# meijieru/AtomNAS

Hardware: AMD Instinct MI355X
Metric: images/sec (whole node) AtomNAS-C supernet 224x224 bs256/GPU (higher is better)
Workload: dtype bf16; 1 GPU; atomnas_c_supernet full training step (fwd + CE-smooth/L2/L1 + bwd + grad all-reduce + RMSprop + EMA), 224x224; per_gpu_batch=256, global_batch=256, parallelism=dp1, hip_graph=True

## Files before the change

### atomnas_amd/_lib.py

```python
import ctypes
import os

_HERE = os.path.dirname(os.path.abspath(__file__))
LIB_PATH = os.environ.get("ATOMNAS_HIP_LIB") or os.path.join(_HERE, "libatomnas_hip.so")

vp, i32, i64, f32, f64, u64 = (ctypes.c_void_p, ctypes.c_int, ctypes.c_long, ctypes.c_float, ctypes.c_double,
                               ctypes.c_ulonglong)

SIGNATURES = {
    "atomnas_dwconv_fwd": [vp, i32, i64, vp, vp, i32, vp, i32, vp, i32, i64, vp, i32, i32, i32, i32, i32, i32, i32, i32, i32, vp],
    "atomnas_dwconv_bwd": [vp, i32, i64, vp, i32, i64, vp, vp, vp, vp, i32, i64, vp, vp, i32, vp, i32, vp, i32, i64, vp, vp, i32, i32,
                           vp, i32, i32, i32, i32, i32, i32, i32, vp],
    "atomnas_pw_gemm_nt": [i32, vp, i32, i64, vp, i32, i64, vp, vp, vp, i32, vp, i32, vp, i32, i64, i32, vp, i32, vp, i32, i64, vp, vp,
                           i32, vp, vp, i32, i32, i64, i32, i32, i32, vp],
    "atomnas_pw_gemm_tn": [i32, vp, i32, i64, vp, i32, i64, vp, vp, vp, i32, i32, i32, vp, i32, i64, vp, i32, i64, vp, vp, vp, i32, i32,
                           vp, i64, i64, i64, vp, i64, i32, vp],
    "atomnas_expand_bwd": [vp, i32, i64, vp, vp, i32, vp, i32, vp, i32, vp, i32, vp, vp, i64, vp, i32, vp, i64, i32, i32, i32, vp],
    "atomnas_project_bwd": [vp, i32, vp, i32, vp, i32, i64, vp, vp, i32, vp, i32, i64, vp, i32, vp, i64, i64, vp, i64, i64, i32, i32, i32, vp],
    "atomnas_bn_finalize_fwd": [vp, i32, i32, f64, vp, vp, f32, f32, vp, vp, vp, vp, vp, vp, vp, i32, vp, vp],
    "atomnas_bn_eval_coeffs": [vp, vp, vp, vp, f32, vp, vp, i32, vp, vp],
    "atomnas_bn_finalize_bwd": [vp, i32, i32, f64, vp, vp, vp, vp, vp, vp, vp, vp, vp, vp, i32, vp, vp],
    "atomnas_bn_apply": [vp, i32, vp, vp, i32, vp, i32, vp, i32, i64, i32, i32, vp],
    "atomnas_bnbwd_apply": [vp, i32, vp, i32, vp, vp, vp, vp, i32, i64, i32, i32, vp],
    "atomnas_bn_act_pool": [vp, i32, vp, vp, i32, vp, i32, vp, f32, u64, vp, i32, i32, i32, i32, vp],
    "atomnas_pool_act_bwd": [vp, i32, vp, f32, vp, i32, vp, vp, i32, vp, i32, vp, i32, i32, i32, i32, i32, vp],
    "atomnas_act_bwd_stats": [vp, i32, vp, i32, vp, vp, i32, vp, i32, vp, i32, i64, i32, i32, vp],
    "atomnas_bn_apply_drop": [vp, i32, vp, vp, vp, i32, vp, i32, vp, f32, u64, vp, i32, i32, i32, i32, i32, vp],
    "atomnas_drop_connect_bwd": [vp, i32, vp, i32, vp, f32, vp, i32, vp, i32, i32, i32, i32, i32, vp],
    "atomnas_se_squeeze": [vp, i32, i64, vp, vp, i32, vp, i32, i32, i64, i32, i32, i32, i32, vp],
    "atomnas_se_mlp_fwd": [vp, i32, i32, i64, vp, vp, vp, vp, vp, vp, i32, vp, vp, i32, i32, i32, vp],
    "atomnas_se_scale": [vp, i32, i64, vp, vp, i32, vp, i32, vp, i32, i64, i64, i32, i32, i32, vp],
    "atomnas_se_bwd_gate": [vp, i32, i64, vp, i32, i64, vp, vp, i32, vp, vp, i32, vp, vp, vp, vp, vp, i32, i64, vp, vp, vp, vp, vp, vp, vp, i32, i32,
                            i32, i32, i32, i32, i32, vp],
    "atomnas_se_bwd_apply": [vp, i32, i64, vp, i32, i64, vp, vp, i32, vp, vp, i32, vp, i32, i64, vp, i32, i64, i32, i32, i32, vp],
    "atomnas_im2col_stem": [vp, vp, i32, i32, i32, i32, i32, vp],
    "atomnas_ce_smooth": [vp, i32, vp, f32, i32, i32, vp, vp, i32, f32, vp, i32, vp],
    "atomnas_colsum": [vp, i32, vp, i64, i32, i32, vp],
    "atomnas_fused_rmsprop_ema": [vp, vp, vp, vp, vp, vp, i64, vp, f64, f64, i32, f64, vp, vp, vp],
    "atomnas_fused_sgd_ema": [vp, vp, vp, vp, vp, i64, vp, f64, i32, vp, vp, vp],
    "atomnas_grad_guard": [vp, i64, vp, f32, i32, vp, vp, vp],
    "atomnas_fused_rmsprop_ema_guarded": [vp, vp, vp, vp, vp, vp, i64, vp, f64, f64, i32, f64, vp, vp, vp, vp],
    "atomnas_fused_sgd_ema_guarded": [vp, vp, vp, vp, vp, i64, vp, f64, i32, vp, vp, vp, vp],
    "atomnas_ema_update_guarded": [vp, vp, i64, vp, vp, vp],
    "atomnas_guard_restore": [vp, vp, i64, vp, i32, vp],
    "atomnas_vec_sum": [vp, i32, f32, vp, vp],
    "atomnas_ema_update": [vp, vp, i64, vp, vp],
    "atomnas_scale_by": [vp, i64, vp, i32, vp],
    "atomnas_accum_fold": [vp, vp, vp, i64, i32, i32, f32, vp],
    "atomnas_zero": [vp, i64, vp],
    "atomnas_add_i64": [vp, i64, i64, vp],
    "atomnas_reg_grad": [vp, vp, vp, i32, i32, vp, vp, vp],
    "atomnas_reg_value": [vp, vp, i32, i32, vp, f32, vp, vp, vp],
    "atomnas_pack_weights": [vp, vp, vp, i32, i32, vp],
    "atomnas_reduce_defer": [i32, vp],
    "atomnas_reduce_flush": [vp],
    "atomnas_gamma_mask": [vp, vp, vp, i32, f32, i32, vp, vp, vp, vp],
    "atomnas_mask_index": [vp, i32, vp, vp, vp],
    "atomnas_gather_dim": [vp, vp, vp, i64, i64, i64, i64, i32, i32, i32, vp],
    "atomnas_gather_jobs": [vp, i32, i64, vp],
    "atomnas_gram": [vp, i32, i64, i32, vp, i64, vp, vp, i32, vp],
    "atomnas_image_preprocess": [vp, vp, i32, i32, vp, vp, vp, i32, i32, vp],
    "atomnas_image_preprocess_large": [vp, vp, vp, i32, i32, i32, vp, vp, vp, i32, i32, vp, i64, vp],
    "atomnas_image_resize_window": [vp, vp, vp, i32, i32, vp, vp, vp, i32, i32, vp],
    "atomnas_image_resize_window_large": [vp, vp, vp, vp, i32, i32, i32, vp, vp, vp, i32, i32, vp, i64, vp],
    "atomnas_image_color": [vp, vp, i32, i32, vp, vp, vp, i32, vp, i32, vp],
    "atomnas_xb_coeffs": [vp, vp, vp, i32, vp, i32, vp, i32, i32, vp, i32, vp, vp, vp],
    "atomnas_fold_jobs": [vp, i32, i32, i64, i64, vp],
    "atomnas_block_infer": [vp, i32, vp, i32, vp, i32, vp, i32, vp, vp, vp, vp, vp, vp, vp, i32, i32, i32, i32, i32, i32, vp, vp, vp, i32, i32,
                            i32, i32, i32, vp],
    "atomnas_block_infer_se": [vp, i32, vp, i32, vp, i32, vp, i32, vp, vp, vp, vp, vp, vp, vp, i32, i32, i32, i32, i32, i32, vp, vp, vp, i32, i32,
                               i32, i32, i32, vp, vp, vp, vp, i32, i32, vp],
}
NO_STATUS = {"atomnas_last_error": (ctypes.c_char_p, []), "atomnas_abi_version": (i32, []),
             "atomnas_runtime_version": (i32, []), "atomnas_grad_guard_ws_floats": (i32, []), "atomnas_expand_bwd_supported": (i32, [i32, i32, i32]),
             "atomnas_project_bwd_supported": (i32, [i32, i32, i32]),
             "atomnas_project_bwd_dp_supported": (i32, [i64, i32, i32, i32, i32, i64, i32, i64, i32, i32]),
             "atomnas_dwconv_cw_supported": (i32, [i32, i32, i32, i32, i32, i32, i32, i32]),
             "atomnas_dwconv_mm_supported": (i32, [i32, i32, i32, i32, i32, i32, i32, i32]),
             "atomnas_se_pool_parts": (i32, [i32, i32, i32]),
             "atomnas_block_infer_supported": (i32, [i32, i32, i32, i32, i32, i32, vp, vp, vp, i32, i32, i32, i32, i32, i32]),
             "atomnas_block_infer_runs": (i32, [i32, i32, i32, i32, i32, i32, vp, vp, vp, i32, i32, i32, i32, i32, i32]),
             "atomnas_block_infer_se_supported": (i32, [i32, i32, i32, i32, i32, i32, vp, vp, vp, i32, i32, i32, i32, i32, i32]),
             "atomnas_block_infer_se_runs": (i32, [i32, i32, i32, i32, i32, i32, vp, vp, vp, i32, i32, i32, i32, i32, i32])}

ABI_VERSION = 9
_lib = None


class AtomnasHipError(RuntimeError):
    pass


def exported_symbols():
    return sorted(list(SIGNATURES) + list(NO_STATUS))


def load():
    global _lib
    if _lib is not None:
        return _lib
    import torch
    if not os.path.exists(LIB_PATH):
        raise AtomnasHipError(
            "libatomnas_hip.so is missing (%s). Build it with `python -m atomnas_amd.build`; there is no CPU fallback." % LIB_PATH)
    lib = ctypes.CDLL(LIB_PATH)
    for name, args in SIGNATURES.items():
        fn = getattr(lib, name)
        fn.argtypes = args
        fn.restype = i32
    for name, (res, args) in NO_STATUS.items():
        fn = getattr(lib, name)
        fn.argtypes = args
        fn.restype = res
    if lib.atomnas_abi_version() != ABI_VERSION:
        raise AtomnasHipError("%s has ABI version %d, this package binds version %d: rebuild with `python -m atomnas_amd.build`"
                              % (LIB_PATH, lib.atomnas_abi_version(), ABI_VERSION))
    _lib = lib
    return lib


PROFILE = None
_TAG = [None]


def profile_tag(tag):
    _TAG[0] = tag


def call(name, *args):
    lib = load()
    if PROFILE is not None:
        import torch
        e0, e1 = torch.cuda.Event(enable_timing=True), torch.cuda.Event(enable_timing=True)
        e0.record()
        rc = getattr(lib, name)(*args)
        e1.record()
        PROFILE.append((name, _TAG[0], e0, e1))
    else:
        rc = getattr(lib, name)(*args)
    if rc != 0:
        raise AtomnasHipError("%s failed (rc=%d): %s" % (name, rc, lib.atomnas_last_error().decode()))
```

### atomnas_amd/csrc/head.hip

```cpp
#include "common.h"

namespace atomnas {

template <typename T>
__global__ __launch_bounds__(256) void k_im2col_stem(const float* __restrict__ img, T* __restrict__ col, int ld, int N, int H, int W,
                                                     int Ho, int Wo) {
  const long total = (long)N * Ho * Wo;
  for (long m = (long)blockIdx.x * 256 + threadIdx.x; m < total; m += (long)gridDim.x * 256) {
    const int wo = (int)(m % Wo), ho = (int)((m / Wo) % Ho), n = (int)(m / ((long)Wo * Ho));
    float v[32];
#pragma unroll
    for (int i = 0; i < 32; ++i) v[i] = 0.f;
#pragma unroll
    for (int ci = 0; ci < 3; ++ci) {
      const float* plane = img + ((long)n * 3 + ci) * H * W;
#pragma unroll
      for (int ky = 0; ky < 3; ++ky) {
        const int hi = 2 * ho + ky - 1;
#pragma unroll
        for (int kx = 0; kx < 3; ++kx) {
          const int wi = 2 * wo + kx - 1;
          if (hi >= 0 && hi < H && wi >= 0 && wi < W) v[ci * 9 + ky * 3 + kx] = plane[(long)hi * W + wi];
        }
      }
    }
    T* o = col + m * ld;
#pragma unroll
    for (int g8 = 0; g8 < 4; ++g8) {
      float t[8];
#pragma unroll
      for (int e = 0; e < 8; ++e) t[e] = v[8 * g8 + e];
      VecIO<T, 8>::store(o + 8 * g8, t);
    }
    const float z8[8] = {0.f, 0.f, 0.f, 0.f, 0.f, 0.f, 0.f, 0.f};
    for (int c = 32; c < ld; c += 8) VecIO<T, 8>::store(o + c, z8);
  }
}

template <typename T>
__global__ __launch_bounds__(256) void k_ce_smooth(const float* __restrict__ logits, int ldl, const long long* __restrict__ target,
                                                   float eps, int B, int K, float* __restrict__ loss_per_sample,
                                                   T* __restrict__ dlogits, int ldd, float gscale,
                                                   int* __restrict__ topk_correct ) {
  const int lane = threadIdx.x & 63;
  const int b = blockIdx.x * 4 + (threadIdx.x >> 6);
  if (b >= B) return;
  const float* x = logits + (long)b * ldl;
  const int y = (int)target[b];
  float mx = -INFINITY;
  for (int j = lane; j < K; j += 64) mx = fmaxf(mx, x[j]);
#pragma unroll
  for (int o = 32; o > 0; o >>= 1) mx = fmaxf(mx, __shfl_xor(mx, o, 64));
  float se = 0.f, sx = 0.f;
  const float xy = x[y];
  int rank = 0;
  for (int j = lane; j < K; j += 64) {
    const float v = x[j];
    se += expf(v - mx);
    sx += v;
    rank += (v > xy) ? 1 : 0;
  }
  se = wave_sum(se);
  sx = wave_sum(sx);
#pragma unroll
  for (int o = 32; o > 0; o >>= 1) rank += __shfl_xor(rank, o, 64);
  const float lse = mx + logf(se);
  const float loss = -(1.f - eps) * (xy - lse) - (eps / (float)K) * (sx - (float)K * lse);
  if (lane == 0) {
    if (loss_per_sample) loss_per_sample[b] = loss;
    if (topk_correct) {
      if (rank < 1) atomicAdd(&topk_correct[0], 1);
      if (rank < 5) atomicAdd(&topk_correct[1], 1);
    }
  }
  if (dlogits) {
    T* d = dlogits + (long)b * ldd;
    const float invB = gscale / (float)B;
    for (int j = lane; j < ldd; j += 64) {
      float g = 0.f;
      if (j < K) {
        const float p = expf(x[j] - lse);
        const float t = eps / (float)K + ((j == y) ? (1.f - eps) : 0.f);
        g = (p - t) * invB;
      }
      d[j] = from_f32<T>(g);
    }
  }
}

template <typename T>
__global__ __launch_bounds__(256) void k_colsum(const T* __restrict__ x, int ld, float* __restrict__ out, long M, int C) {
  const int c = blockIdx.x * 256 + threadIdx.x;
  if (c >= C) return;
  float s0 = 0.f, s1 = 0.f, s2 = 0.f, s3 = 0.f;
  long m = 0;
  for (; m + 3 < M; m += 4) {
    s0 += to_f32(x[m * ld + c]);
    s1 += to_f32(x[(m + 1) * ld + c]);
    s2 += to_f32(x[(m + 2) * ld + c]);
    s3 += to_f32(x[(m + 3) * ld + c]);
  }
  for (; m < M; ++m) s0 += to_f32(x[m * ld + c]);
  out[c] += (s0 + s1) + (s2 + s3);
}

}

using namespace atomnas;

extern "C" int atomnas_im2col_stem(const float* img, void* col, int ld, int N, int H, int W, int dtype, void* stream) {
  ATOMNAS_REQUIRE(img && col && ld >= 32 && ld % 8 == 0 && N > 0 && H > 0 && W > 0, "im2col_stem: bad arguments");
  const int Ho = (H + 2 - 3) / 2 + 1, Wo = (W + 2 - 3) / 2 + 1;
  const long total = (long)N * Ho * Wo;
  long blocks = (total + 255) / 256;
  if (blocks > 8192) blocks = 8192;
  hipStream_t st = (hipStream_t)stream;
  if (dtype == DT_F32)
    hipLaunchKernelGGL(k_im2col_stem<float>, dim3((unsigned)blocks), dim3(256), 0, st, img, (float*)col, ld, N, H, W, Ho, Wo);
  else
    hipLaunchKernelGGL(k_im2col_stem<bf16_t>, dim3((unsigned)blocks), dim3(256), 0, st, img, (bf16_t*)col, ld, N, H, W, Ho, Wo);
  return check_launch("im2col_stem");
}

extern "C" int atomnas_ce_smooth(const float* logits, int ldl, const long long* target, float eps, int B, int K, float* loss_per_sample,
                                 void* dlogits, int ldd, float gscale, int* topk_correct, int dtype, void* stream) {
  ATOMNAS_REQUIRE(logits && target && B > 0 && K > 0 && ldl >= K, "ce_smooth: bad arguments");
  ATOMNAS_REQUIRE(!dlogits || ldd >= K, "ce_smooth: bad gradient pitch");
  hipStream_t st = (hipStream_t)stream;
  if (dtype == DT_F32)
    hipLaunchKernelGGL(k_ce_smooth<float>, dim3((B + 3) / 4), dim3(256), 0, st, logits, ldl, target, eps, B, K, loss_per_sample,
                       (float*)dlogits, ldd, gscale, topk_correct);
  else
    hipLaunchKernelGGL(k_ce_smooth<bf16_t>, dim3((B + 3) / 4), dim3(256), 0, st, logits, ldl, target, eps, B, K, loss_per_sample,
                       (bf16_t*)dlogits, ldd, gscale, topk_correct);
  return check_launch("ce_smooth");
}

extern "C" int atomnas_colsum(const void* x, int ld, float* out, long M, int C, int dtype, void* stream) {
  ATOMNAS_REQUIRE(x && out && M > 0 && C > 0 && ld >= C, "colsum: bad arguments");
  dim3 grid((C + 255) / 256);
  hipStream_t st = (hipStream_t)stream;
  if (dtype == DT_F32) hipLaunchKernelGGL(k_colsum<float>, grid, dim3(256), 0, st, (const float*)x, ld, out, M, C);
  else hipLaunchKernelGGL(k_colsum<bf16_t>, grid, dim3(256), 0, st, (const bf16_t*)x, ld, out, M, C);
  return check_launch("colsum");
}
```

### atomnas_amd/functional.py

```python
import os

import torch
from torch import nn

from . import ops
from .ops import PRO_BNBWD, PRO_BNRELU, PRO_NONE, STAT_SQ, STAT_Z
from .ops import Slab
from .runtime import pad8, pads

ACT_NONE, ACT_RELU, ACT_RELU6, ACT_SWISH = 0, 1, 2, 3


def act_code(module):
    if module is None:
        return ACT_NONE
    if isinstance(module, nn.ReLU6):
        return ACT_RELU6
    if isinstance(module, nn.ReLU):
        return ACT_RELU
    if type(module).__name__ == "Swish":
        return ACT_SWISH
    raise NotImplementedError("activation %s is not supported by the HIP path (ReLU / ReLU6 / Swish)" % type(module).__name__)


# ... 367 lines not shown
    @staticmethod
    def backward(ctx, gout):
        pl, sv = ctx.pl, ctx.sv
        G, _ = to_2d(gout, pl.mgr.compute_dtype)
        N, H, W, _, _ = sv["dims"]
        gx = block_backward(pl, sv, G)
        _stap(pl, gx=gx)
        ctx.sv = None
        pl.mgr.grad_done(pl)
        return to_4d(gx, N, H, W, pl.inp), None, None


def run_block(pl, x, anchor):
    if pl.nb == 0:
        return x
    if torch.is_grad_enabled() and (x.requires_grad or anchor.requires_grad):
        return BlockFunction.apply(x, anchor, pl)
    x2d, (N, H, W, C) = to_2d(x, pl.mgr.compute_dtype)
    out, _ = block_forward(pl, x2d, N, H, W, False)
    s = pl.stride
    return to_4d(out, N, (H - 1) // s + 1, (W - 1) // s + 1, pl.oup)


class SEFunction(torch.autograd.Function):

    @staticmethod
    def forward(ctx, x, w1, b1, w2, b2, se_act, dtype):
        x2d, (N, H, W, C) = to_2d(x, dtype)
        dev = x.device
        hid = w1.shape[0]
        HT = pads(C)
        M = N * H * W
        D = ops.zeros(M, HT, dtype=dtype, device=dev)
        D[:, :C] = x2d
        cmap = torch.full((HT,), -1, dtype=torch.int32, device=dev)
        cmap[:C] = torch.arange(C, dtype=torch.int32, device=dev)
        w1p, w2t, b2p = (ops.zeros(*shape, dtype=torch.float32, device=dev) for shape in ((hid, HT), (hid, HT), (HT,)))
        w1p[:, :C] = w1.detach().reshape(hid, C).float()
        w2t[:, :C] = w2.detach().reshape(C, hid).float().t()
        b2p[:C] = b2.detach().float()
        one, zero = torch.ones(HT, dtype=torch.float32, device=dev), ops.zeros(HT, dtype=torch.float32, device=dev)
        one[C:] = 0
        S = torch.empty(M, HT, dtype=dtype, device=dev)
        sv = _se_forward(D, one, zero, ACT_NONE, S, cmap, w1p, b1.detach().float().contiguous(), w2t, b2p, se_act, hid, N, H * W, HT)
        ctx.save_for_backward(D, one, zero, sv["gate"], sv["pooled"], cmap, w1p, w2t, sv["hpre"])
        ctx.dims = (N, H, W, C, HT, hid, se_act, dtype)
        return to_4d(S[:, :C], N, H, W, C)

    @staticmethod
    def backward(ctx, gout):
        D, one, zero, gate, pooled, cmap, w1p, w2t, hpre = ctx.saved_tensors
        N, H, W, C, HT, hid, se_act, dtype = ctx.dims
        dev = D.device
        M = N * H * W
        g2d, _ = to_2d(gout, dtype)
        dS = ops.zeros(M, HT, dtype=dtype, device=dev)
        dS[:, :C] = g2d
        dw1, db1, dw2, db2 = (_f32(hid * C, dev, zero=True), _f32(hid, dev, zero=True), _f32(C * hid, dev, zero=True), _f32(C, dev, zero=True))
        g = torch.empty(M, HT, dtype=dtype, device=dev)
        _se_backward(dS, D, one, zero, ACT_NONE, dict(gate=gate, pooled=pooled, hpre=hpre), cmap, w1p, w2t, se_act, hid, dw1, db1, dw2, db2,
                     C, g, _stats(HT, dev), N, H * W, HT)
        return (to_4d(g[:, :C], N, H, W, C), dw1.view(hid, C, 1, 1), db1, dw2.view(C, hid, 1, 1), db2, None, None)


def run_se(module, x):
    dtype = x.dtype if x.dtype in (torch.float32, torch.bfloat16) else torch.float32
    return SEFunction.apply(x, module.se_reduce.weight, module.se_reduce.bias, module.se_expand.weight, module.se_expand.bias,
                            act_code(module.active_fn), dtype)


def convbn_forward(pl, x, need_grad):
    mgr = pl.mgr
    T = mgr.compute_dtype
    dev = x.device
    act = pl.act
    sv = {}
    if pl.groups == 1 and pl.k == 3:
        if pl.cin != 3 or pl.stride != 2:
            raise NotImplementedError("dense 3x3 convolution other than the 3-channel stride-2 stem")
        N, _, H, W = x.shape
        Ho, Wo = (H - 1) // 2 + 1, (W - 1) // 2 + 1
        M = N * Ho * Wo
        col = torch.empty(M, 32, dtype=T, device=dev)
        ops.im2col_stem(x.float().contiguous(), col, N, H, W)
        a2d, K = col, 27
        sv["kind"] = "stem"
    elif pl.groups == 1 and pl.k == 1:
        a2d, (N, H, W, C) = to_2d(x, T)
        Ho, Wo, M, K = H, W, N * H * W, pl.cin
        sv["kind"] = "pw"
    else:
        a2d, (N, H, W, C) = to_2d(x, T)
        s = pl.stride
        Ho, Wo = (H - 1) // s + 1, (W - 1) // s + 1
        M = N * Ho * Wo
        sv["kind"] = "dw"
    Cp = pad8(pl.cout)
    Y = torch.empty(M, Cp, dtype=T, device=dev) if sv["kind"] != "dw" else ops.zeros(M, Cp, dtype=T, device=dev)
    st = _stats(pl.cout, dev, pl.bn["mgr"]) if bn_uses_batch_stats(pl.bn) else None
    if sv["kind"] == "dw":
        ops.dwconv_fwd(a2d, None, None, 0, pl.taps, Y, stat_ld=pl.cout, N=N, H=H, W=W, C=pl.cout, k=pl.k, stride=pl.stride,
                       **_fwd_stats(st, mode=False))
    else:
        ops.gemm_nt(a2d, pl.W_pack, Y, M, pl.cout, K, **_fwd_stats(st))
    b = bn_forward_coeffs(pl.bn, st, M, dev)
    if act:
        _tap("convbn", pl, Y, b)
    out = torch.empty(M, Cp, dtype=T, device=dev)
    ops.bn_apply(Y, b.scale, b.shift, int(act), None, out, M, pl.cout)
    _stap(pl, Y=Y, bn=b, out=out)
    if need_grad:
        sv.update(a=a2d, Y=Y, b=b, dims=(N, H, W, Ho, Wo), K=K if sv["kind"] != "dw" else 0)
    return out, (N, Ho, Wo), sv


def convbn_backward(pl, sv, G, need_input_grad):
    dev, T = G.device, G.dtype
    N, H, W, Ho, Wo = sv["dims"]
    M = N * Ho * Wo
    act = pl.act
    Y, b, a2d = sv["Y"], sv["b"], sv["a"]
    g = torch.empty_like(Y)
    st2 = _stats(pl.cout, dev, pl.bn["mgr"])
    ops.act_bwd_stats(G, Y, b.scale if act else None, b.shift if act else None, int(act), g, st2.t, M, pl.cout, stat_rows=st2.rows)
    c1, c2, c3 = bn_backward_coeffs(pl.bn, b, st2, M, dev)
    _stap(pl, g=g, c=(c1, c2, c3))
    if sv["kind"] == "dw":
        h = ops.zeros(N * H * W, pad8(pl.cout), dtype=T, device=dev)
        ops.dwconv_bwd(g, Y, c1, c2, c3, a2d, None, None, 0, pl.taps, h, pl.W_grad, None, 0, N, H, W, pl.cout, pl.k, pl.stride)
        return h
    K = sv["K"]
    ops.gemm_tn(a2d, K, g, pl.cout, pl.W_grad, 1, K, M, v_mode=PRO_BNBWD, v2=Y, vc1=c1, vc2=c2, vc3=c3)
    if not need_input_grad or sv["kind"] == "stem":
        return None
    Gx = torch.empty(M, pad8(K), dtype=T, device=dev)
    ops.gemm_nt(g, pl.WT_pack, Gx, M, K, pl.cout, a_mode=PRO_BNBWD, a2=Y, ac1=c1, ac2=c2, ac3=c3)
    return Gx


class ConvBNFunction(torch.autograd.Function):
    @staticmethod
    def forward(ctx, x, anchor, pl):
        out, (N, Ho, Wo), sv = convbn_forward(pl, x, True)
        ctx.pl, ctx.sv = pl, sv
        ctx.x_needs = x.requires_grad
        return to_4d(out[:, :pl.cout] if out.shape[1] != pl.cout else out, N, Ho, Wo, pl.cout)

    @staticmethod
    def backward(ctx, gout):
        pl, sv = ctx.pl, ctx.sv
        G, _ = to_2d(gout, pl.mgr.compute_dtype)
        gx = convbn_backward(pl, sv, G, ctx.x_needs)
        ctx.sv = None
        pl.mgr.grad_done(pl)
        N, H, W, _, _ = sv["dims"]
        if gx is None:
            return None, None, None
        cin = pl.cin
        return to_4d(gx[:, :cin] if gx.shape[1] != cin else gx, N, H, W, cin), None, None


def run_convbn(pl, x, anchor):
    if pl.cout % 8 != 0:
        raise ValueError("ConvBNReLU output channels must be a multiple of 8 on the HIP path, got %d" % pl.cout)
    if torch.is_grad_enabled() and (x.requires_grad or anchor.requires_grad):
        return ConvBNFunction.apply(x, anchor, pl)
    out, (N, Ho, Wo), _ = convbn_forward(pl, x, False)
    return to_4d(out, N, Ho, Wo, pl.cout)


def tail_forward(lp, fp, x, drop_p, training, seed, step_ptr, need_grad):
    mgr = lp.mgr
    T = mgr.compute_dtype
    dev = x.device
    a2d, (N, H, W, C) = to_2d(x, T)
    M = N * H * W
    act = lp.act
    L = torch.empty(M, lp.cout, dtype=T, device=dev)
    st = _stats(lp.cout, dev, lp.bn["mgr"]) if bn_uses_batch_stats(lp.bn) else None
    ops.gemm_nt(a2d, lp.W_pack, L, M, lp.cout, lp.cin, **_fwd_stats(st))
    b = bn_forward_coeffs(lp.bn, st, M, dev)
    if act:
        _tap("convbn", lp, L, b)
    pooled = torch.empty(N, lp.cout, dtype=T, device=dev)
    p = float(drop_p) if training else 0.0
# ... 118 lines not shown
```

### atomnas_amd/ops.py

```python
import ctypes

import os

import torch

from . import _lib
from ._lib import call

PRO_NONE, PRO_BNRELU, PRO_BNBWD = 0, 1, 2
STAT_NONE, STAT_SQ, STAT_Z = 0, 1, 2
HYP_LR, HYP_RHO, HYP_EMA_DECAY, HYP_GRAD_SCALE = 0, 1, 2, 3


RECORD = None


def _lay(t):
    if t is None:
        return None
    return "slab" if isinstance(t, Slab) else int(t.stride(0))


def _rec(entry, **kw):
    if RECORD is not None:
# ... 357 lines not shown
         _p(p_scale), _p(p_shift), int(N), int(H), int(W), int(inp), int(oup), n, _ints(seg_off), _ints(seg_ch), _ints(seg_k), int(stride), int(act),
         int(bool(expand)), int(bool(residual)), dt_code(x.dtype), *se_args, _stream())


def bnbwd_apply(g, x, c1, c2, c3, y, M, C):
    _chk_cuda(g, x, y)
    _rec("bnbwd_apply", M=int(M), C=int(C), g=_lay(g), x=_lay(x), y=_lay(y), dt=dt_code(g.dtype))
    call("atomnas_bnbwd_apply", _p(g), _ld(g), _p(x), _ld(x), _p(c1), _p(c2), _p(c3), _p(y), _ld(y), M, C, dt_code(g.dtype), _stream())


def bn_act_pool(x, scale, shift, relu, pooled, keep, drop_p, seed, step_ptr, N, HW, C):
    _rec("bn_act_pool", N=int(N), HW=int(HW), C=int(C), x=_lay(x), act=int(relu), drop_p=float(drop_p), keep=keep is not None, dt=dt_code(x.dtype))
    call("atomnas_bn_act_pool", _p(x), _ld(x), _p(scale), _p(shift), int(relu), _p(pooled), _ld(pooled), _p(keep), float(drop_p),
         int(seed) & 0xFFFFFFFFFFFFFFFF, _p(step_ptr), N, HW, C, dt_code(x.dtype), _stream())


def pool_act_bwd(dpooled, keep, drop_p, x, scale, shift, relu, g, stats2, N, HW, C, stat_rows=None):
    _rec("pool_act_bwd", N=int(N), HW=int(HW), C=int(C), x=_lay(x), act=int(relu), drop_p=float(drop_p), keep=keep is not None,
         stat_rows=_rows(stats2, stat_rows), dt=dt_code(x.dtype))
    call("atomnas_pool_act_bwd", _p(dpooled), _ld(dpooled), _p(keep), float(drop_p), _p(x), _ld(x), _p(scale), _p(shift), int(relu),
         _p(g), _ld(g), _p(stats2), _rows(stats2, stat_rows), N, HW, C, dt_code(x.dtype), _stream())


def act_bwd_stats(dy, z, scale, shift, relu, g, stats2, M, C, stat_rows=None):
    _rec("act_bwd_stats", M=int(M), C=int(C), dy=_lay(dy), z=_lay(z), masked=scale is not None, act=int(relu), g=_lay(g), stat_rows=_rows(stats2, stat_rows),
         dt=dt_code(dy.dtype))
    call("atomnas_act_bwd_stats", _p(dy), _ld(dy), _p(z), _ld(z), _p(scale), _p(shift), int(relu), _p(g),
         _ld(g) if g is not None else 0, _p(stats2), _rows(stats2, stat_rows), M, C, dt_code(dy.dtype), _stream())


def bn_apply_drop(x, scale, shift, res, y, keep_out, drop_p, seed, step_ptr, block_index, N, HW, C):
    _chk_cuda(x, res, y, keep_out)
    _rec("bn_apply_drop", N=int(N), HW=int(HW), C=int(C), x=_lay(x), res=_lay(res), y=_lay(y), drop_p=float(drop_p), block=int(block_index),
         dt=dt_code(x.dtype))
    call("atomnas_bn_apply_drop", _p(x), _ld(x), _p(scale), _p(shift), _p(res), _ld(res) if res is not None else 0, _p(y), _ld(y), _p(keep_out), float(drop_p),
         int(seed) & 0xFFFFFFFFFFFFFFFF, _p(step_ptr), int(block_index), N, HW, C, dt_code(x.dtype), _stream())


def drop_connect_bwd(g, z, keep, drop_p, gs, stats2, N, HW, C, stat_rows=None):
    _chk_cuda(g, z, keep, gs)
    _rec("drop_connect_bwd", N=int(N), HW=int(HW), C=int(C), g=_lay(g), z=_lay(z), gs=_lay(gs), drop_p=float(drop_p),
         stat_rows=_rows(stats2, stat_rows), dt=dt_code(g.dtype))
    call("atomnas_drop_connect_bwd", _p(g), _ld(g), _p(z), _ld(z), _p(keep), float(drop_p), _p(gs), _ld(gs), _p(stats2),
         _rows(stats2, stat_rows), N, HW, C, dt_code(g.dtype), _stream())


def se_pool_parts(N, HW, C):
    return int(_lib.load().atomnas_se_pool_parts(int(N), int(HW), int(C)))


def se_squeeze(d, scale, shift, act, pooled_parts, N, HW, C):
    parts = pooled_parts.shape[0]
    call("atomnas_se_squeeze", _p(d), _ld(d), _ss(d), _p(scale), _p(shift), int(act), _p(pooled_parts), pooled_parts.stride(1), parts,
         pooled_parts.stride(0), N, HW, C, dt_code(d.dtype), _stream())


def se_mlp_fwd(pooled_parts, pooled, cmap, w1p, b1, w2t, b2p, act, hpre, gate, N, HT, hid):
    call("atomnas_se_mlp_fwd", _p(pooled_parts), pooled_parts.stride(1), pooled_parts.shape[0], pooled_parts.stride(0), _p(pooled), _p(cmap),
         _p(w1p), _p(b1), _p(w2t), _p(b2p), int(act), _p(hpre), _p(gate), N, HT, hid, _stream())


def se_scale(d, scale, shift, act, gate, out, M, HW, C):
    call("atomnas_se_scale", _p(d), _ld(d), _ss(d), _p(scale), _p(shift), int(act), _p(gate), gate.stride(0), _p(out), _ld(out), _ss(out), M,
         HW, C, dt_code(d.dtype), _stream())


def se_bwd_gate(ds, d, scale, shift, act, gate, pooled, cmap, w1p, w2t, hpre,
                dgate, dz2, dz1, dpooled, dw1, db1, dw2, db2, N, HW, HT, total,
                hid, se_act=None):
    call("atomnas_se_bwd_gate", _p(ds), _ld(ds), _ss(ds), _p(d), _ld(d), _ss(d), _p(scale), _p(shift), int(act), _p(gate), _p(pooled),
         gate.stride(0), _p(cmap), _p(w1p), _p(w2t), _p(hpre), _p(dgate), dgate.shape[0], dgate.stride(0), _p(dz2), _p(dz1), _p(dpooled), _p(dw1), _p(db1), _p(dw2), _p(db2),
         int(act if se_act is None else se_act), N, HW, HT, total, hid, dt_code(d.dtype), _stream())


def se_bwd_apply(ds, d, scale, shift, act, gate, dpooled, g, stats2, M, HW, C, stat_rows=None):
    call("atomnas_se_bwd_apply", _p(ds), _ld(ds), _ss(ds), _p(d), _ld(d), _ss(d), _p(scale), _p(shift), int(act), _p(gate), _p(dpooled),
         gate.stride(0), _p(g), _ld(g), _ss(g), _p(stats2), _rows(stats2, stat_rows), M, HW, C, dt_code(d.dtype), _stream())


def im2col_stem(img, col, N, H, W):
    assert img.dtype == torch.float32 and img.is_contiguous()
    _rec("im2col_stem", N=int(N), H=int(H), W=int(W), col=_lay(col), dt=dt_code(col.dtype))
    call("atomnas_im2col_stem", _p(img), _p(col), _ld(col), N, H, W, dt_code(col.dtype), _stream())


def ce_smooth(logits, target, eps, B, K, loss_per_sample, dlogits, gscale, topk):
    assert logits.dtype == torch.float32 and target.dtype == torch.int64
    _rec("ce_smooth", B=int(B), K=int(K), ldl=_lay(logits), dl=_lay(dlogits), dt=dt_code(dlogits.dtype) if dlogits is not None else 0)
    call("atomnas_ce_smooth", _p(logits), _ld(logits), _p(target), float(eps), B, K, _p(loss_per_sample), _p(dlogits),
         _ld(dlogits) if dlogits is not None else 0, float(gscale), _p(topk),
         dt_code(dlogits.dtype) if dlogits is not None else 0, _stream())


def colsum(x, out, M, C):
    _rec("colsum", M=int(M), C=int(C), x=_lay(x), dt=dt_code(x.dtype))
    call("atomnas_colsum", _p(x), _ld(x), _p(out), M, C, dt_code(x.dtype), _stream())


def fused_rmsprop_ema(p, g, sq, buf, ema, wd_chunk, n, hyper, alpha, eps, eps_inside_sqrt, momentum, l2_value=None, ws=None, guard=None):
    if l2_value is not None and ws is None:
        ws = torch.empty(4096, dtype=torch.float32, device=p.device)
    args = (_p(p), _p(g), _p(sq), _p(buf), _p(ema), _p(wd_chunk), n, _p(hyper), float(alpha), float(eps), int(eps_inside_sqrt),
            float(momentum), _p(l2_value), _p(ws))
    if guard is None:
        call("atomnas_fused_rmsprop_ema", *args, _stream())
    else:
        call("atomnas_fused_rmsprop_ema_guarded", *args, _p(guard), _stream())


def fused_sgd_ema(p, g, buf, ema, wd_chunk, n, hyper, momentum, nesterov, l2_value=None, ws=None, guard=None):
    if l2_value is not None and ws is None:
        ws = torch.empty(4096, dtype=torch.float32, device=p.device)
    args = (_p(p), _p(g), _p(buf), _p(ema), _p(wd_chunk), n, _p(hyper), float(momentum), int(bool(nesterov)), _p(l2_value), _p(ws))
    if guard is None:
        call("atomnas_fused_sgd_ema", *args, _stream())
    else:
        call("atomnas_fused_sgd_ema_guarded", *args, _p(guard), _stream())


GUARD_OK, GUARD_SCALE, GUARD_NORM, GUARD_COEF, GUARD_SKIPPED, GUARD_CLIPPED = 0, 1, 2, 3, 4, 5
GUARD_WORDS = 8


def grad_guard_ws_floats():
    return int(_lib.load().atomnas_grad_guard_ws_floats())


def grad_guard(g, n, hyper, max_norm, skip_nonfinite, guard, ws=None):
    if ws is None:
        ws = torch.empty(grad_guard_ws_floats(), dtype=torch.float32, device=g.device)
    assert guard.dtype == torch.float32 and guard.numel() >= GUARD_WORDS and ws.numel() >= grad_guard_ws_floats()
    call("atomnas_grad_guard", _p(g), int(n), _p(hyper), float(max_norm), int(bool(skip_nonfinite)), _p(ws), _p(guard), _stream())


def ema_update_guarded(shadow, x, n, hyper, guard):
    call("atomnas_ema_update_guarded", _p(shadow), _p(x), n, _p(hyper), _p(guard), _stream())


def guard_restore(dst, src, n, guard, unconditional=False):
    call("atomnas_guard_restore", _p(dst), _p(src), int(n), _p(guard), int(bool(unconditional)), _stream())


def vec_sum(x, n, scale, out):
    call("atomnas_vec_sum", _p(x), int(n), float(scale), _p(out), _stream())


def ema_update(shadow, x, n, hyper):
    call("atomnas_ema_update", _p(shadow), _p(x), n, _p(hyper), _stream())


def zero_(t):
    if isinstance(t, Slab):
        zero_(t.t)
        return t
    assert t.is_contiguous()
    if t.numel():
        call("atomnas_zero", _p(t), t.numel() * t.element_size(), _stream())
    return t


def zeros(*shape, dtype, device):
    return zero_(torch.empty(*shape, dtype=dtype, device=device))


def add_i64(t, v):
    assert t.dtype == torch.int64 and t.is_contiguous()
# ... 147 lines not shown
```

### include/atomnas_hip.h

```cpp
#ifndef ATOMNAS_HIP_H
#define ATOMNAS_HIP_H

#ifdef __cplusplus
extern "C" {
#endif

#define ATOMNAS_STAT_ROWS_DEFAULT 512

#define ATOMNAS_DT_F32 0
#define ATOMNAS_DT_BF16 1

#define ATOMNAS_ACT_NONE 0
#define ATOMNAS_ACT_RELU 1
#define ATOMNAS_ACT_RELU6 2
#define ATOMNAS_ACT_SWISH 3

#define ATOMNAS_PRO_NONE 0
#define ATOMNAS_PRO_BNRELU 1
#define ATOMNAS_PRO_BNBWD 2

#define ATOMNAS_STAT_NONE 0
#define ATOMNAS_STAT_SQ 1
#define ATOMNAS_STAT_Z 2

// ... 15 lines not shown
int atomnas_runtime_version(void);

int atomnas_dwconv_fwd(const void* x, int ldx, long x_ss, const float* in_scale, const float* in_shift, int in_relu, const float* w,
                       int ldw, void* y, int ldy, long y_ss, float* stats, int stat_ld, int stat_rows, int N, int H, int W, int C, int k, int stride,
                       int dtype, void* stream);

int atomnas_dwconv_bwd(const void* g, int ldg, long g_ss, const void* yraw, int ldyr, long yraw_ss, const float* c1, const float* c2,
                       const float* c3, const void* x, int ldx, long x_ss, const float* in_scale, const float* in_shift, int in_relu,
                       const float* w, int ldw, void* h, int ldh, long h_ss, float* dw, float* stats, int stat_ld, int part_rows, float* dw_ws, int N, int H, int W,
                       int C, int k, int stride, int dtype, void* stream);

int atomnas_dwconv_cw_supported(int N, int H, int W, int C, int k, int stride, int dtype, int dir);

int atomnas_dwconv_mm_supported(int N, int H, int W, int C, int k, int stride, int dtype, int dir);

int atomnas_pw_gemm_nt(int a_mode, const void* a, int lda, long a_ss, const void* a2, int lda2, long a2_ss, const float* ac1,
                       const float* ac2, const float* ac3, int a_relu, const void* wp, int ldw, void* c, int ldc, long c_ss, int out_f32,
                       const void* add, int ldadd, const void* z, int ldz, long z_ss, const float* zscale, const float* zshift, int mask, const float* bias,
                       float* stats, int stat_mode, int stat_rows, long M, int N, int K, int dtype, void* stream);

int atomnas_pw_gemm_tn(int u_mode, const void* u, int ldu, long u_ss, const void* u2, int ldu2, long u2_ss, const float* uc1,
                       const float* uc2, const float* uc3, int u_relu, int NU, int v_mode, const void* v, int ldv, long v_ss,
                       const void* v2, int ldv2, long v2_ss, const float* vc1, const float* vc2, const float* vc3, int v_relu, int NV, float* out, long si, long sj, long M,
                       float* ws, long ws_floats, int dtype, void* stream);

int atomnas_expand_bwd_supported(int inp, int hid, int dtype);
int atomnas_expand_bwd(const void* h, int ldh, long h_ss, const float* c1, const void* x, int ldx, const void* wt, int ldw, const void* add,
                       int ldadd, void* gx, int ldgx, float* dwe, float* ws, long ws_floats, const void* mp, int ldm, const float* vb, long M,
                       int inp, int hid, int dtype, void* stream);
int atomnas_gram(const void* x, int ldx, long M, int inp, float* ws, long ws_floats, float* gram, float* sx, int dtype, void* stream);
int atomnas_xb_coeffs(const float* c2, const float* c3, const void* wexp, int ldwe, const float* gram, int ldg, const float* sx, int inp,
                      int C, void* mp, int ldm, float* vb, float* dwe, void* stream);

int atomnas_project_bwd_supported(int oup, int hid, int dtype);
int atomnas_project_bwd_dp_supported(long M, int oup, int hid, int ldg, int ldz, long z_ss, int ldgh, long gh_ss, int stat_rows, int dtype);
int atomnas_project_bwd(const void* g, int ldg, const void* wpt, int ldw, const void* z, int ldz, long z_ss, const float* zscale,
                        const float* zshift, int act, void* gh, int ldgh, long gh_ss, float* stats, int stat_rows, float* dwp, long si,
                        long sj, float* ws, long ws_floats, long M, int oup, int hid, int dtype, void* stream);

int atomnas_bn_finalize_fwd(const float* stats, int stat_rows, int stat_ld, double count, const float* gamma, const float* beta, float eps, float momentum,
                            float* running_mean, float* running_var, long long* num_batches_tracked, float* scale, float* shift,
                            float* save_mean, float* save_invstd, int C, const int* cmap, void* stream);
int atomnas_bn_eval_coeffs(const float* gamma, const float* beta, const float* running_mean, const float* running_var, float eps,
                           float* scale, float* shift, int C, const int* cmap, void* stream);
int atomnas_bn_finalize_bwd(const float* stats2, int stat_rows, int stat_ld, double count, const float* gamma, const float* save_mean, const float* save_invstd,
                            const float* rho_ptr, const float* penalty, float* dgamma, float* dbeta, float* c1, float* c2, float* c3,
                            int C, const int* cmap, void* stream);
int atomnas_bn_apply(const void* x, int ldx, const float* scale, const float* shift, int relu, const void* res, int ldres, void* y,
                     int ldy, long M, int C, int dtype, void* stream);
int atomnas_bnbwd_apply(const void* g, int ldg, const void* x, int ldx, const float* c1, const float* c2, const float* c3, void* y,
                        int ldy, long M, int C, int dtype, void* stream);
int atomnas_bn_act_pool(const void* x, int ldx, const float* scale, const float* shift, int relu, void* pooled, int ldp,
                        unsigned char* keep, float drop_p, unsigned long long seed, const long long* step_ptr, int N, int HW, int C,
                        int dtype, void* stream);
int atomnas_pool_act_bwd(const void* dpooled, int ldp, const unsigned char* keep, float drop_p, const void* x, int ldx,
                         const float* scale, const float* shift, int relu, void* g, int ldg, float* stats2, int stat_rows, int N,
                         int HW, int C, int dtype, void* stream);
int atomnas_act_bwd_stats(const void* dy, int lddy, const void* z, int ldz, const float* scale, const float* shift, int relu, void* g,
                          int ldg, float* stats2, int stat_rows, long M, int C, int dtype, void* stream);
int atomnas_bn_apply_drop(const void* x, int ldx, const float* scale, const float* shift, const void* res, int ldres, void* y, int ldy,
                          unsigned char* keep_out, float drop_p, unsigned long long seed, const long long* step_ptr, int block_index,
                          int N, int HW, int C, int dtype, void* stream);
int atomnas_drop_connect_bwd(const void* g, int ldg, const void* z, int ldz, const unsigned char* keep, float drop_p, void* gs, int ldgs,
                             float* stats2, int stat_rows, int N, int HW, int C, int dtype, void* stream);

int atomnas_se_pool_parts(int N, int HW, int C);
int atomnas_se_squeeze(const void* d, int ldd, long d_ss, const float* scale, const float* shift, int act, float* pooled_parts, int ldp,
                       int parts, long part_stride, int N, int HW, int C, int dtype, void* stream);
int atomnas_se_mlp_fwd(const float* pooled_parts, int ldp, int parts, long part_stride, float* pooled, const int* cmap, const float* w1p,
                       const float* b1, const float* w2t, const float* b2p, int act, float* hpre, float* gate, int N, int HT, int hid,
                       void* stream);
int atomnas_se_scale(const void* d, int ldd, long d_ss, const float* scale, const float* shift, int act, const float* gate, int ldg,
                     void* out, int ldo, long o_ss, long M, int HW, int C, int dtype, void* stream);
int atomnas_se_bwd_gate(const void* ds, int ldds, long ds_ss, const void* d, int ldd, long d_ss, const float* scale, const float* shift,
                        int act, const float* gate, const float* pooled, int ldg, const int* cmap, const float* w1p, const float* w2t,
                        const float* hpre, float* dgate, int parts, long part_stride, float* dz2, float* dz1, float* dpooled, float* dw1,
                        float* db1, float* dw2,
                        float* db2, int se_act, int N, int HW, int HT, int total, int hid, int dtype, void* stream);
int atomnas_se_bwd_apply(const void* ds, int ldds, long ds_ss, const void* d, int ldd, long d_ss, const float* scale, const float* shift,
                         int act, const float* gate, const float* dpooled, int ldg, void* g, int ldgo, long g_ss, float* stats2,
                         int stat_rows, long M, int HW, int C, int dtype, void* stream);

int atomnas_im2col_stem(const float* img, void* col, int ld, int N, int H, int W, int dtype, void* stream);
int atomnas_ce_smooth(const float* logits, int ldl, const long long* target, float eps, int B, int K, float* loss_per_sample,
                      void* dlogits, int ldd, float gscale, int* topk_correct, int dtype, void* stream);
int atomnas_colsum(const void* x, int ld, float* out, long M, int C, int dtype, void* stream);

int atomnas_fused_rmsprop_ema(float* p, const float* g, float* sq, float* buf, float* ema, const float* wd_chunk, long n,
                              const float* hyper, double alpha, double eps, int eps_inside_sqrt, double momentum, float* l2_value,
                              float* ws, void* stream);
int atomnas_fused_sgd_ema(float* p, const float* g, float* buf, float* ema, const float* wd_chunk, long n, const float* hyper,
                          double momentum, int nesterov, float* l2_value, float* ws, void* stream);
int atomnas_grad_guard_ws_floats(void);
int atomnas_grad_guard(const float* g, long n, const float* hyper, float max_norm, int skip_nonfinite, float* ws, float* guard, void* stream);
int atomnas_fused_rmsprop_ema_guarded(float* p, const float* g, float* sq, float* buf, float* ema, const float* wd_chunk, long n,
                                      const float* hyper, double alpha, double eps, int eps_inside_sqrt, double momentum, float* l2_value,
                                      float* ws, const float* guard, void* stream);
int atomnas_fused_sgd_ema_guarded(float* p, const float* g, float* buf, float* ema, const float* wd_chunk, long n, const float* hyper,
                                  double momentum, int nesterov, float* l2_value, float* ws, const float* guard, void* stream);
int atomnas_ema_update_guarded(float* shadow, const float* x, long n, const float* hyper, const float* guard, void* stream);
int atomnas_guard_restore(float* dst, const float* src, long n, const float* guard, int unconditional, void* stream);
int atomnas_vec_sum(const float* x, int n, float scale, float* out, void* stream);
int atomnas_ema_update(float* shadow, const float* x, long n, const float* hyper, void* stream);
int atomnas_scale_by(float* x, long n, const float* hyper, int idx, void* stream);
int atomnas_accum_fold(float* acc, float* cur, const float* base, long n, int first, int last, float inv_count, void* stream);
int atomnas_zero(void* p, long bytes, void* stream);
int atomnas_add_i64(long* p, long n, long v, void* stream);
int atomnas_reg_grad(const float* p, float* g, const void* jobs_dev, int njobs, int use_sign, const float* mult_ptr,
                     const float* grad_out_ptr, void* stream);
int atomnas_reg_value(const float* p, const void* jobs_dev, int njobs, int use_abs, const float* mult_ptr, float post_scale,
                      float* out, float* ws , void* stream);
int atomnas_pack_weights(const float* arena, void* packbuf, const void* jobs_dev, int njobs, int dtype, void* stream);

typedef struct atomnas_img_desc {
  long off;
  int H, W;
  int bi, bj, bh, bw;
  int flip;
  int pad_;
} atomnas_img_desc;
int atomnas_image_preprocess(const void* pool, const void* desc, int N, int S, const float* mean3, const float* std3, void* out,
                             int out_mode, int filter, void* stream);
int atomnas_image_preprocess_large(const void* pool, const void* desc, const int* sel, int M, int max_rows, int S, const float* mean3,
                                   const float* std3, void* out, int out_mode, int filter, void* workspace, long workspace_bytes,
                                   void* stream);

typedef struct atomnas_img_aug {
  int oh, ow;
  int top, left;
  int op[3];
  int pad_;
  float factor[3];
  float pad2_;
  double inc[3];
} atomnas_img_aug;
int atomnas_image_resize_window(const void* pool, const void* desc, const void* aug, int N, int S, const float* mean3, const float* std3,
                                void* out, int out_mode, int filter, void* stream);
int atomnas_image_resize_window_large(const void* pool, const void* desc, const void* aug, const int* sel, int M, int max_rows, int S,
                                      const float* mean3, const float* std3, void* out, int out_mode, int filter, void* workspace,
                                      long workspace_bytes, void* stream);
int atomnas_image_color(const void* src, const void* aug, int N, int S, const float* mean3, const float* std3, void* out, int out_mode,
                        void* means, int form, void* stream);

int atomnas_reduce_defer(int on, void* stream);
int atomnas_reduce_flush(void* stream);

typedef struct atomnas_fold_job {
  float* src;
  float* dst;
  long src_ld, dst_ld;
  int rows, cols;
  unsigned blk0;
  int pad_;
} atomnas_fold_job;
int atomnas_fold_jobs(const void* jobs_dev, int first, int njobs, long blk_base, long nblocks, void* stream);

int atomnas_gamma_mask(const float* params, const float* ema, const void* jobs_dev, int njobs, float threshold, int mode,
                       unsigned char* mask, int* index, int* kept, void* stream);
int atomnas_mask_index(const unsigned char* mask, int count, int* index, int* kept, void* stream);
int atomnas_gather_dim(const float* src, float* dst, const int* index, long src_os, long src_ds, long dst_os, long dst_ds, int outer,
                       int n_kept, int inner, void* stream);
typedef struct atomnas_gather_job {
  const float* src;
  float* dst;
  const int* index;
  long src_os, src_ds, dst_os, dst_ds;
// ... 30 lines not shown
```

Baseline: 9887 images/sec.

## Fuse stem im2col, GEMM and BN statistics into one stem conv kernel

Adds a dedicated stem convolution kernel that gathers 3x3 stride-2 patches straight from the fp32 image with buffer loads and runs them through bf16 MFMA against the packed weights. It writes the col buffer, which backward still needs, along with the output, and accumulates BN statistics in the same pass. The kernel is persistent and software-prefetches the next tile. This removes the separate im2col launch and the GEMM's re-read of the col matrix from memory. The generic im2col plus GEMM path is kept as a fallback when the shape or dtype is unsupported. The stem is a small part of the whole training step, so the effect on the full step is likely minor.

```diff
diff --git a/atomnas_amd/_lib.py b/atomnas_amd/_lib.py
--- a/atomnas_amd/_lib.py
+++ b/atomnas_amd/_lib.py
@@ -34,6 +34,7 @@
                             i32, i32, i32, i32, i32, vp],
     "atomnas_se_bwd_apply": [vp, i32, i64, vp, i32, i64, vp, vp, i32, vp, vp, i32, vp, i32, i64, vp, i32, i64, i32, i32, i32, vp],
     "atomnas_im2col_stem": [vp, vp, i32, i32, i32, i32, i32, vp],
+    "atomnas_stem_conv_fwd": [vp, vp, i32, vp, i32, vp, i32, vp, i32, i32, i32, i32, i32, i32, vp],
     "atomnas_ce_smooth": [vp, i32, vp, f32, i32, i32, vp, vp, i32, f32, vp, i32, vp],
     "atomnas_colsum": [vp, i32, vp, i64, i32, i32, vp],
     "atomnas_fused_rmsprop_ema": [vp, vp, vp, vp, vp, vp, i64, vp, f64, f64, i32, f64, vp, vp, vp],
@@ -75,6 +76,7 @@
              "atomnas_runtime_version": (i32, []), "atomnas_grad_guard_ws_floats": (i32, []), "atomnas_expand_bwd_supported": (i32, [i32, i32, i32]),
              "atomnas_project_bwd_supported": (i32, [i32, i32, i32]),
              "atomnas_project_bwd_dp_supported": (i32, [i64, i32, i32, i32, i32, i64, i32, i64, i32, i32]),
+             "atomnas_stem_conv_fwd_supported": (i32, [i32, i32, i32, i32, i32, i32]),
              "atomnas_dwconv_cw_supported": (i32, [i32, i32, i32, i32, i32, i32, i32, i32]),
              "atomnas_dwconv_mm_supported": (i32, [i32, i32, i32, i32, i32, i32, i32, i32]),
              "atomnas_se_pool_parts": (i32, [i32, i32, i32]),
diff --git a/atomnas_amd/csrc/head.hip b/atomnas_amd/csrc/head.hip
--- a/atomnas_amd/csrc/head.hip
+++ b/atomnas_amd/csrc/head.hip
@@ -1,4 +1,4 @@
-#include "common.h"
+#include "pwconv.h"
 
 namespace atomnas {
 
@@ -34,6 +34,148 @@
     }
     const float z8[8] = {0.f, 0.f, 0.f, 0.f, 0.f, 0.f, 0.f, 0.f};
     for (int c = 32; c < ld; c += 8) VecIO<T, 8>::store(o + c, z8);
+  }
+}
+
+constexpr int STEM_TP = 2;
+constexpr unsigned STEM_OOB = 0x80000000u;
+typedef __attribute__((ext_vector_type(4))) unsigned stem_u32x4;
+typedef __attribute__((ext_vector_type(2))) unsigned stem_u32x2;
+
+__global__ __launch_bounds__(256) void k_stem_conv_fwd(const float* __restrict__ img, const bf16_t* __restrict__ Wp, int ldw,
+                                                       bf16_t* __restrict__ col, bf16_t* __restrict__ Y, int ldy, float* __restrict__ stats,
+                                                       int stat_rows, int M, int H, int W, int Ho, int Wo, unsigned img_bytes) {
+  using MM = Mma<bf16_t>;
+  constexpr int SWD = 64;
+  __shared__ float s_stat[8 * SWD];
+  const int tid = threadIdx.x;
+  const int lane = tid & 63, wave = tid >> 6;
+  const int q = lane >> 4, j = lane & 15;
+  const bool do_stats = stats != nullptr;
+  if (do_stats) {
+    for (int i = tid; i < 8 * SWD; i += 256) s_stat[i] = 0.f;
+    __syncthreads();
+  }
+  bf16x8 wf[2];
+#pragma unroll
+  for (int t = 0; t < 2; ++t) wf[t] = MM::raw(Wp + (long)(j + 16 * t) * ldw + 8 * q);
+
+  int toff[8];
+  unsigned mK = 0, mT = 0, mB = 0, mL = 0, mR = 0;
+#pragma unroll
+  for (int e = 0; e < 8; ++e) {
+    const int k = 8 * q + e;
+    const int ci = k / 9, ky = (k % 9) / 3, kx = k % 3;
+    toff[e] = ((ci * H + (ky - 1)) * W + (kx - 1)) * 4;
+    if (k >= 27) mK |= 1u << e;
+    if (ky == 0) mT |= 1u << e;
+    if (ky == 2) mB |= 1u << e;
+    if (kx == 0) mL |= 1u << e;
+    if (kx == 2) mR |= 1u << e;
+  }
+  const __amdgpu_buffer_rsrc_t rimg = __builtin_amdgcn_make_buffer_rsrc(const_cast<float*>(img), 0, (int)img_bytes, 0x00020000);
+  const __amdgpu_buffer_rsrc_t rcol = __builtin_amdgcn_make_buffer_rsrc(col, 0, M * 64, 0x00020000);
+  const __amdgpu_buffer_rsrc_t ry = __builtin_amdgcn_make_buffer_rsrc(Y, 0, M * ldy * 2, 0x00020000);
+
+  const int mtiles = (M + 15) / 16;
+  const int stride = (int)gridDim.x * 4 * STEM_TP;
+  const int dwo = (stride * 16) % Wo, dho = (stride * 16 / Wo) % Ho, dn = stride * 16 / Wo / Ho;
+  int prow[STEM_TP], pn[STEM_TP], pho[STEM_TP], pwo[STEM_TP];
+  int mt = ((int)blockIdx.x * 4 + wave) * STEM_TP;
+#pragma unroll
+  for (int u = 0; u < STEM_TP; ++u) {
+    const int row = (mt + u) * 16 + j;
+    prow[u] = row;
+    pwo[u] = row % Wo;
+    pho[u] = (row / Wo) % Ho;
+    pn[u] = row / Wo / Ho;
+  }
+  float nx[STEM_TP][8];
+  auto fetch = [&]() {
+#pragma unroll
+    for (int u = 0; u < STEM_TP; ++u) {
+      const int ho = pho[u], wo = pwo[u];
+      const unsigned base = (((unsigned)pn[u] * 3u * (unsigned)H + 2u * (unsigned)ho) * (unsigned)W + 2u * (unsigned)wo) * 4u;
+      const unsigned inv = mK | (ho == 0 ? mT : 0u) | (2 * ho + 1 >= H ? mB : 0u) | (wo == 0 ? mL : 0u) | (2 * wo + 1 >= W ? mR : 0u) |
+                           (prow[u] >= M ? 0xffu : 0u);
+#pragma unroll
+      for (int e = 0; e < 8; ++e)
+        nx[u][e] = __builtin_bit_cast(float, __builtin_amdgcn_raw_buffer_load_b32(rimg, (inv >> e) & 1u ? STEM_OOB : base + (unsigned)toff[e], 0, 0));
+      prow[u] += stride * 16;
+      int w2 = wo + dwo;
+      const int cw = w2 >= Wo;
+      w2 -= cw ? Wo : 0;
+      int h2 = ho + dho + cw;
+      const int ch = h2 >= Ho;
+      h2 -= ch ? Ho : 0;
+      pwo[u] = w2;
+      pho[u] = h2;
+      pn[u] += dn + ch;
+    }
+  };
+
+  float s1[8], s2[8];
+#pragma unroll
+  for (int i = 0; i < 8; ++i) s1[i] = s2[i] = 0.f;
+  fetch();
+#pragma unroll
+  for (int u = 0; u < STEM_TP; ++u) {
+    __builtin_amdgcn_raw_buffer_store_b128(stem_u32x4{0u, 0u, 0u, 0u}, rcol, STEM_OOB, 0, 0);
+    __builtin_amdgcn_raw_buffer_store_b64(stem_u32x2{0u, 0u}, ry, STEM_OOB, 0, 0);
+    __builtin_amdgcn_raw_buffer_store_b64(stem_u32x2{0u, 0u}, ry, STEM_OOB, 0, 0);
+  }
+  for (; mt < mtiles; mt += stride) {
+    float cur[STEM_TP][8];
+#pragma unroll
+    for (int u = 0; u < STEM_TP; ++u)
+#pragma unroll
+      for (int e = 0; e < 8; ++e) cur[u][e] = nx[u][e];
+    fetch();
+#pragma unroll
+    for (int u = 0; u < STEM_TP; ++u) {
+      const int row = (mt + u) * 16 + j;
+      const bool rowvalid = row < M;
+      const bf16x8 af = MM::pack(cur[u]);
+      __builtin_amdgcn_raw_buffer_store_b128(__builtin_bit_cast(stem_u32x4, af), rcol, rowvalid ? (unsigned)(row * 64 + 16 * q) : STEM_OOB, 0, 0);
+#pragma unroll
+      for (int t = 0; t < 2; ++t) {
+        const f32x4 acc = MM::mma(wf[t], af, f32x4{0.f, 0.f, 0.f, 0.f});
+        bf16x4 ob;
+#pragma unroll
+        for (int r = 0; r < 4; ++r) ob[r] = (bf16_t)acc[r];
+        stem_u32x2 bits = __builtin_bit_cast(stem_u32x2, ob);
+        asm volatile("" : "+v"(bits));
+        const f32x2 lo = bf16_pair_f32(bits[0]), hi = bf16_pair_f32(bits[1]);
+        __builtin_amdgcn_raw_buffer_store_b64(bits, ry, rowvalid ? (unsigned)((row * ldy + 16 * t + 4 * q) * 2) : STEM_OOB, 0, 0);
+        const float c[4] = {lo[0], lo[1], hi[0], hi[1]};
+#pragma unroll
+        for (int r = 0; r < 4; ++r) {
+          s1[4 * t + r] += c[r];
+          s2[4 * t + r] += c[r] * c[r];
+        }
+      }
+    }
+  }
+  if (do_stats) {
+    float* sw = s_stat + wave * 2 * SWD;
+#pragma unroll
+    for (int i = 0; i < 8; ++i) {
+      float a = s1[i], b = s2[i];
+#pragma unroll
+      for (int o = 8; o > 0; o >>= 1) {
+        a += __shfl_xor(a, o, 64);
+        b += __shfl_xor(b, o, 64);
+      }
+      const int ch = 16 * (i >> 2) + 4 * q + (i & 3);
+      if (j == 0) {
+        sw[ch] = a;
+        sw[SWD + ch] = b;
+      }
+    }
+    Epilogue ep = {};
+    ep.stats = stats;
+    ep.stat_rows = stat_rows;
+    nt_flush_stats(ep, s_stat, SWD, 0, 32, blockIdx.x, gridDim.x, tid);
   }
 }
 
@@ -122,6 +264,32 @@
   return check_launch("im2col_stem");
 }
 
+extern "C" int atomnas_stem_conv_fwd_supported(int cout, int ldcol, int N, int H, int W, int dtype) {
+  if (cout != 32 || ldcol != 32 || dtype != DT_BF16 || N <= 0 || H <= 0 || W <= 0) return 0;
+  const long Ho = (H - 1) / 2 + 1, Wo = (W - 1) / 2 + 1;
+  return (long)N * 3 * H * W * 4 < (1L << 31) && (long)N * Ho * Wo * 64 < (1L << 30);
+}
+
+extern "C" int atomnas_stem_conv_fwd(const float* img, const void* wp, int ldw, void* col, int ldcol, void* y, int ldy, float* stats,
+                                     int stat_rows, int N, int H, int W, int cout, int dtype, void* stream) {
+  ATOMNAS_REQUIRE(img && wp && col && y && ldw >= 32 && ldw % 8 == 0, "stem_conv_fwd: bad arguments");
+  ATOMNAS_REQUIRE(atomnas_stem_conv_fwd_supported(cout, ldcol, N, H, W, dtype),
+                  "stem_conv_fwd: no instance for cout=%d ldcol=%d N=%d H=%d W=%d dtype=%d (atomnas_im2col_stem + atomnas_pw_gemm_nt serve it)", cout,
+                  ldcol, N, H, W, dtype);
+  ATOMNAS_REQUIRE(ldy >= 32 && ldy <= 64 && ldy % 8 == 0, "stem_conv_fwd: bad output pitch %d", ldy);
+  ATOMNAS_REQUIRE(!stats || stat_rows > 0, "stem_conv_fwd: statistics without partial rows");
+  const int Ho = (H - 1) / 2 + 1, Wo = (W - 1) / 2 + 1;
+  const int M = N * Ho * Wo;
+  const long steps = ((M + 15) / 16 + 4 * STEM_TP - 1) / (4 * STEM_TP);
+  long R = (long)num_cus() * resident_per_cu(k_stem_conv_fwd, 256, 0);
+  if (R > steps) R = steps;
+  if (stats && R > stat_rows) R = stat_rows;
+  if (R < 1) R = 1;
+  hipLaunchKernelGGL(k_stem_conv_fwd, dim3((unsigned)R), dim3(256), 0, (hipStream_t)stream, img, (const bf16_t*)wp, ldw, (bf16_t*)col,
+                     (bf16_t*)y, ldy, stats, stat_rows, M, H, W, Ho, Wo, (unsigned)((long)N * 3 * H * W * 4));
+  return check_launch("stem_conv_fwd");
+}
+
 extern "C" int atomnas_ce_smooth(const float* logits, int ldl, const long long* target, float eps, int B, int K, float* loss_per_sample,
                                  void* dlogits, int ldd, float gscale, int* topk_correct, int dtype, void* stream) {
   ATOMNAS_REQUIRE(logits && target && B > 0 && K > 0 && ldl >= K, "ce_smooth: bad arguments");
diff --git a/atomnas_amd/functional.py b/atomnas_amd/functional.py
--- a/atomnas_amd/functional.py
+++ b/atomnas_amd/functional.py
@@ -473,7 +473,10 @@
         Ho, Wo = (H - 1) // 2 + 1, (W - 1) // 2 + 1
         M = N * Ho * Wo
         col = torch.empty(M, 32, dtype=T, device=dev)
-        ops.im2col_stem(x.float().contiguous(), col, N, H, W)
+        img = x.float().contiguous()
+        stem_fused = ops.stem_conv_fwd_supported(pl.cout, col, N, H, W)
+        if not stem_fused:
+            ops.im2col_stem(img, col, N, H, W)
         a2d, K = col, 27
         sv["kind"] = "stem"
     elif pl.groups == 1 and pl.k == 1:
@@ -492,6 +495,8 @@
     if sv["kind"] == "dw":
         ops.dwconv_fwd(a2d, None, None, 0, pl.taps, Y, stat_ld=pl.cout, N=N, H=H, W=W, C=pl.cout, k=pl.k, stride=pl.stride,
                        **_fwd_stats(st, mode=False))
+    elif sv["kind"] == "stem" and stem_fused:
+        ops.stem_conv_fwd(img, pl.W_pack, col, Y, N, H, W, pl.cout, **_fwd_stats(st, mode=False))
     else:
         ops.gemm_nt(a2d, pl.W_pack, Y, M, pl.cout, K, **_fwd_stats(st))
     b = bn_forward_coeffs(pl.bn, st, M, dev)
diff --git a/atomnas_amd/ops.py b/atomnas_amd/ops.py
--- a/atomnas_amd/ops.py
+++ b/atomnas_amd/ops.py
@@ -463,6 +463,21 @@
     assert img.dtype == torch.float32 and img.is_contiguous()
     _rec("im2col_stem", N=int(N), H=int(H), W=int(W), col=_lay(col), dt=dt_code(col.dtype))
     call("atomnas_im2col_stem", _p(img), _p(col), _ld(col), N, H, W, dt_code(col.dtype), _stream())
+
+
+def stem_conv_fwd_supported(cout, col, N, H, W):
+    return bool(_lib.load().atomnas_stem_conv_fwd_supported(int(cout), _ld(col), int(N), int(H), int(W), dt_code(col.dtype)))
+
+
+def stem_conv_fwd(img, wp, col, y, N, H, W, cout, stats=None, stat_rows=None):
+    _chk_cuda(img, wp, col, y)
+    assert img.dtype == torch.float32 and img.is_contiguous()
+    if _lib.PROFILE is not None:
+        _lib.profile_tag("N%d H%d W%d" % (N, H, W))
+    _rec("stem_conv_fwd", N=int(N), H=int(H), W=int(W), cout=int(cout), ldw=int(wp.stride(0)), col=_lay(col), y=_lay(y),
+         stat_rows=_rows(stats, stat_rows), dt=dt_code(col.dtype))
+    call("atomnas_stem_conv_fwd", _p(img), _p(wp), wp.stride(0), _p(col), _ld(col), _p(y), _ld(y), _p(stats), _rows(stats, stat_rows),
+         N, H, W, int(cout), dt_code(col.dtype), _stream())
 
 
 def ce_smooth(logits, target, eps, B, K, loss_per_sample, dlogits, gscale, topk):
diff --git a/include/atomnas_hip.h b/include/atomnas_hip.h
--- a/include/atomnas_hip.h
+++ b/include/atomnas_hip.h
@@ -121,6 +121,9 @@
                          int stat_rows, long M, int HW, int C, int dtype, void* stream);
 
 int atomnas_im2col_stem(const float* img, void* col, int ld, int N, int H, int W, int dtype, void* stream);
+int atomnas_stem_conv_fwd_supported(int cout, int ldcol, int N, int H, int W, int dtype);
+int atomnas_stem_conv_fwd(const float* img, const void* wp, int ldw, void* col, int ldcol, void* y, int ldy, float* stats, int stat_rows,
+                          int N, int H, int W, int cout, int dtype, void* stream);
 int atomnas_ce_smooth(const float* logits, int ldl, const long long* target, float eps, int B, int K, float* loss_per_sample,
                       void* dlogits, int ldd, float gscale, int* topk_correct, int dtype, void* stream);
 int atomnas_colsum(const void* x, int ld, float* out, long M, int C, int dtype, void* stream);
```

Result: no change. 9908 images/sec (median of 6 runs) (+0.2%).
